# iacopoermacora/Street-sparse-3DGS

Hardware: AMD Instinct MI355X
Metric: fwd+bwd Mpix/s at 1080p (1M Gaussians) (higher is better)
Workload: dtype f32; 1 GPU; rasterizer fwd+bwd, 1000000 Gaussians, SH degree 3, 1920x1080, do_depth; gaussians=1000000, width=1920, height=1080, sh_degree=3, tiles=8160, fwd_segment=2048, parallelism=chunk-per-gpu x1

## Files before the change

### street-sparse-3dgs_amd/csrc/dsort.hip

```cpp
#include "gsr_launch.h"

namespace gsr {

namespace {

constexpr int kDsThreads = 1024;
constexpr int kDsWaves = kDsThreads / kWave;
constexpr int kDsItems = 8;
constexpr int kDsTile = kDsThreads * kDsItems;
constexpr int kRadix = 256;
constexpr int kPasses = 4;
constexpr int kLookWin = 16;
constexpr int kMaxResident = 240;

constexpr int kCtlTicket = 0;
constexpr int kCtlDone = 4;
constexpr int kCtlK = 5;
constexpr int kCtlErr = 6;
constexpr int kCtlAux = 7;
constexpr int kCtlMaxSB = 8;
constexpr int kCtlFwdReady = 9;
constexpr int kCtlLongest = 10;
constexpr int kCtlCulled = 12;
constexpr int kCtlLive = 13;
constexpr int kCtlHead = 16;
constexpr int kUpMax = 128;
__host__ __device__ inline int up_tpb(int nb) { return (nb + kUpMax - 1) / kUpMax; }
__host__ __device__ inline int up_blocks(int nb) { return (nb + up_tpb(nb) - 1) / up_tpb(nb); }
__host__ __device__ inline size_t ctl_status(int nb, int p) { return kCtlHead + (size_t)p * nb * kRadix; }
__host__ __device__ inline size_t ctl_zero_words(int nb) { return ctl_status(nb, kPasses); }
__host__ __device__ inline size_t ctl_bex(int nb) { return ctl_zero_words(nb); }
__host__ __device__ inline size_t ctl_btot(int nb) { return ctl_bex(nb) + nb; }
__host__ __device__ inline size_t ctl_blkhist(int nb) { return (ctl_btot(nb) + kUpMax + 63) / 64 * 64; }
__host__ __device__ inline size_t ctl_words(int nb) { return ctl_blkhist(nb) + (size_t)kUpMax * kPasses * kRadix; }
constexpr int kSpinLimit = 1 << 20;

#ifdef GSR_DS_TRACE
__device__ uint64_t *g_ds_trace;
#define DS_STAMP(kern, slot)                                                                          \
    do {                                                                                              \
        if (threadIdx.x == 0) {                                                                       \
// ... 22 lines not shown
#endif

constexpr uint32_t kFlagAgg = 1u << 30, kFlagInc = 2u << 30, kCountMask = (1u << 30) - 1u;

__device__ __forceinline__ uint32_t ld_agent(const uint32_t *p) {
    return __hip_atomic_load(p, __ATOMIC_RELAXED, __HIP_MEMORY_SCOPE_AGENT);
}
__device__ __forceinline__ void st_agent(uint32_t *p, uint32_t v) {
    __hip_atomic_store(p, v, __ATOMIC_RELAXED, __HIP_MEMORY_SCOPE_AGENT);
}

__device__ __forceinline__ uint32_t below(uint64_t m) {
    return __builtin_amdgcn_mbcnt_hi((uint32_t)(m >> 32), __builtin_amdgcn_mbcnt_lo((uint32_t)m, 0u));
}

__device__ __forceinline__ uint64_t match8(uint32_t d, uint64_t valid) {
    uint64_t m = valid;
#pragma unroll
    for (int b = 0; b < 8; b++) {
        const bool bit = (d >> b) & 1u;
        const uint64_t bb = __ballot(bit);
        m &= bit ? bb : ~bb;
    }
    return m;
}

__device__ __forceinline__ uint32_t wave_incl_scan(uint32_t v, int lane) {
#pragma unroll
    for (int o = 1; o < 64; o <<= 1) {
        const uint32_t t = (uint32_t)__shfl_up((int)v, o, 64);
        if (lane >= o) v += t;
    }
    return v;
}

__device__ __forceinline__ uint32_t scan256_wave(uint32_t *a, int lane) {
    const uint32_t x0 = a[4 * lane], x1 = a[4 * lane + 1], x2 = a[4 * lane + 2], x3 = a[4 * lane + 3];
    const uint32_t s = x0 + x1 + x2 + x3;
    const uint32_t incl = wave_incl_scan(s, lane);
    const uint32_t e = incl - s;
    a[4 * lane] = e;
    a[4 * lane + 1] = e + x0;
    a[4 * lane + 2] = e + x0 + x1;
    a[4 * lane + 3] = e + x0 + x1 + x2;
    return (uint32_t)__shfl((int)incl, 63, 64);
}

__global__ __launch_bounds__(kDsThreads) void dsort_upsweep_kernel(int P, int nb, const uint32_t *__restrict__ keys,
                                                                    const uint32_t *__restrict__ tiles,
                                                                    uint32_t *__restrict__ ctl,
                                                                    uint32_t *__restrict__ host_K) {
    GSR_KS(kKsUpsweep);
    constexpr int kTopCopies = 16;
    __shared__ uint32_t s_hist[kPasses * kRadix];
    __shared__ uint32_t s_top[kTopCopies][kRadix];
    __shared__ uint32_t s_mid[kTopCopies][kRadix];
    __shared__ uint32_t s_wsum[kDsWaves];
    __shared__ uint32_t s_cull;
    const int t = threadIdx.x, w = t >> 6, lane = t & 63;
    const int u = blockIdx.x, tpb = up_tpb(nb);
    DS_STAMP(0, 0);
    s_hist[t] = 0u;
    if (t == 0) s_cull = 0u;
#pragma unroll
    for (int k = 0; k < kTopCopies * kRadix / kDsThreads; k++) {
        (&s_top[0][0])[t + k * kDsThreads] = 0u;
        (&s_mid[0][0])[t + k * kDsThreads] = 0u;
    }
    __syncthreads();
    uint32_t run = 0;
    uint32_t culled = 0;
    const int v1 = min(nb, (u + 1) * tpb);
    for (int v = u * tpb; v < v1; v++) {
        const size_t base = (size_t)v * kDsTile + (size_t)w * kDsItems * kWave;
        uint32_t key[kDsItems], tl[kDsItems];
#pragma unroll
        for (int k = 0; k < kDsItems; k++) {
            const size_t e = base + (size_t)k * kWave + lane;
            key[k] = e < (size_t)P ? keys[e] : 0u;
            tl[k] = e < (size_t)P ? tiles[e] : 0u;
        }
        uint32_t sum = 0;
#pragma unroll
        for (int k = 0; k < kDsItems; k++) {
            const size_t e = base + (size_t)k * kWave + lane;
            const bool cull = e < (size_t)P && key[k] == 0xFFFFFFFFu;
            culled += (uint32_t)__popcll(__ballot(cull));
            if (e < (size_t)P && !cull) {
#pragma unroll
                for (int p = 0; p < kPasses - 2; p++) atomicAdd(&s_hist[p * kRadix + ((key[k] >> (8 * p)) & 0xFFu)], 1u);
                atomicAdd(&s_mid[lane & (kTopCopies - 1)][(key[k] >> 16) & 0xFFu], 1u);
                atomicAdd(&s_top[lane & (kTopCopies - 1)][key[k] >> 24], 1u);
            }
            sum += tl[k];
        }
#pragma unroll
        for (int o = 32; o > 0; o >>= 1) sum += (uint32_t)__shfl_xor((int)sum, o, 64);
        if (lane == 0) s_wsum[w] = sum;
        __syncthreads();
        if (t == 0) {
            ctl[ctl_bex(nb) + v] = run;
#pragma unroll
            for (int k = 0; k < kDsWaves; k++) run += s_wsum[k];
        }
        __syncthreads();
    }
    if (lane == 0 && culled) atomicAdd(&s_cull, culled);
    __syncthreads();
    DS_STAMP(0, 1);
    uint32_t hv = s_hist[t];
    if (t >= (kPasses - 1) * kRadix) {
#pragma unroll
        for (int c = 0; c < kTopCopies; c++) hv += s_top[c][t - (kPasses - 1) * kRadix];
    } else if (t >= (kPasses - 2) * kRadix) {
#pragma unroll
        for (int c = 0; c < kTopCopies; c++) hv += s_mid[c][t - (kPasses - 2) * kRadix];
    }
    ctl[ctl_blkhist(nb) + (size_t)u * kPasses * kRadix + t] = hv;
    if (t == 0) {
        ctl[ctl_btot(nb) + u] = run;
        __hip_atomic_fetch_add(&ctl[kCtlK], run, __ATOMIC_RELAXED, __HIP_MEMORY_SCOPE_AGENT);
        if (s_cull) __hip_atomic_fetch_add(&ctl[kCtlCulled], s_cull, __ATOMIC_RELAXED, __HIP_MEMORY_SCOPE_AGENT);
        const uint32_t done = __hip_atomic_fetch_add(&ctl[kCtlDone], 1u, __ATOMIC_ACQ_REL, __HIP_MEMORY_SCOPE_AGENT);
        if (done == (uint32_t)gridDim.x - 1u && host_K) {
            const uint32_t K = ld_agent(&ctl[kCtlK]);
            __hip_atomic_store(host_K, K, __ATOMIC_RELAXED, __HIP_MEMORY_SCOPE_SYSTEM);
        }
    }
    DS_STAMP(0, 2);
}

template <int kPass>
__global__ __launch_bounds__(kDsThreads) void dsort_pass_kernel(int P, int nb, const uint32_t *__restrict__ kin,
                                                                 uint32_t *__restrict__ kout,
                                                                 const uint32_t *__restrict__ vin,
                                                                 uint32_t *__restrict__ vout, uint32_t *__restrict__ ctl,
                                                                 uint32_t *__restrict__ offsets,
                                                                 const uint32_t *__restrict__ tiles,
                                                                 const uint2 *__restrict__ rect8,
                                                                 const uint32_t *__restrict__ rect4,
                                                                 uint2 *__restrict__ drect,
                                                                 const uint32_t *__restrict__ rin,
                                                                 uint32_t *__restrict__ rout,
                                                                 uint32_t *__restrict__ host_err) {
    GSR_KS(kKsPass0 + kPass);
    constexpr bool kFirst = kPass == 0, kLast = kPass == kPasses - 1;
    const bool carry = GSR_DSORT_CARRY && rect4 != nullptr;
    constexpr int kShift = 8 * kPass;
    __shared__ uint32_t s_key[kDsTile];
    __shared__ uint32_t s_val[kDsTile];
    __shared__ uint32_t s_rc[GSR_DSORT_CARRY ? kDsTile : 1];
    __shared__ uint32_t s_wh[kDsWaves][kRadix];
    __shared__ uint32_t s_gb[4][kRadix];
    __shared__ uint32_t s_bex[kRadix];
    __shared__ uint32_t s_dst[kRadix];
    __shared__ uint32_t s_wsum[kDsWaves];
    __shared__ uint32_t s_v, s_pre, s_nsort;
    const int t = threadIdx.x, w = t >> 6, lane = t & 63;
    DS_STAMP(1 + kPass, 0);
#pragma unroll
    for (int k = 0; k < kDsWaves * kRadix / kDsThreads; k++) (&s_wh[0][0])[t + k * kDsThreads] = 0u;
    const int nbu = up_blocks(nb);
    uint32_t h[kUpMax / 4];
    {
        const uint32_t *bh = ctl + ctl_blkhist(nb) + kPass * kRadix + (t & (kRadix - 1));
#pragma unroll
        for (int q = 0; q < kUpMax / 4; q++) {
            const int j = (t >> 8) + 4 * q;
            h[q] = j < nbu ? bh[(size_t)j * kPasses * kRadix] : 0u;
        }
    }
    uint32_t v = blockIdx.x;
    if (nb > kMaxResident) {
        if (t == 0) s_v = atomicAdd(&ctl[kCtlTicket + kPass], 1u);
        __syncthreads();
        v = s_v;
    } else {
        __builtin_amdgcn_s_waitcnt(0xc07f);
        __builtin_amdgcn_s_barrier();
    }
    const size_t Pn = kFirst ? (size_t)P : (size_t)P - min((size_t)ctl[kCtlCulled], (size_t)P);
    const uint32_t nbv = (uint32_t)((Pn + kDsTile - 1) / kDsTile);
    if (v >= nbv) return;
    DS_STAMP(1 + kPass, 5);
    const int wbase = w * kDsItems * kWave;
    const size_t tile0 = (size_t)v * kDsTile;
    const int n = (int)min((size_t)kDsTile, Pn - tile0);
    uint32_t key[kDsItems], val[kDsItems], tl[kDsItems], rc[kDsItems];
    const uint32_t *rsrc = kFirst ? rect4 : rin;
#pragma unroll
    for (int k = 0; k < kDsItems; k++) {
        const int i = wbase + k * kWave + lane;
        const bool valid = i < n;
        key[k] = valid ? kin[tile0 + i] : 0xFFFFFFFFu;
        val[k] = kFirst ? (uint32_t)(tile0 + i) : (valid ? vin[tile0 + i] : 0u);
        tl[k] = (kFirst && valid) ? tiles[tile0 + i] : 0u;
        rc[k] = (!kFirst && carry && valid) ? rsrc[tile0 + i] : 0u;
    }
    DS_STAMP_AFTER(1 + kPass, 6, key[kDsItems - 1] + val[kDsItems - 1]);
    uint32_t toff[kDsItems];
    if (kFirst) {
        if (w == 0) {
            const int u = (int)v / up_tpb(nb);
            uint32_t c = 0;
#pragma unroll
            for (int q = 0; q < kUpMax / kWave; q++) c += lane + q * kWave < u ? ctl[ctl_btot(nb) + lane + q * kWave] : 0u;
#pragma unroll
            for (int o = 32; o > 0; o >>= 1) c += (uint32_t)__shfl_xor((int)c, o, 64);
            if (lane == 0) s_pre = c + ctl[ctl_bex(nb) + v];
        }
        uint32_t run = 0;
#pragma unroll
        for (int k = 0; k < kDsItems; k++) {
            const uint32_t incl = wave_incl_scan(tl[k], lane);
            toff[k] = run + incl - tl[k];
            run += (uint32_t)__shfl((int)incl, 63, 64);
        }
        if (lane == 0) s_wsum[w] = run;
    }
    uint32_t rk[kDsItems];
#pragma unroll
    for (int k = 0; k < kDsItems; k++) {
        const bool valid = wbase + k * kWave + lane < n && key[k] != 0xFFFFFFFFu;
        const uint32_t d = (key[k] >> kShift) & 0xFFu;
        const uint64_t m = match8(d, __ballot(valid));
        const uint32_t b = below(m);
        const uint32_t old = s_wh[w][d];
        if (valid && b == 0u) s_wh[w][d] = old + (uint32_t)__popcll(m);
        rk[k] = old + b;
    }
    {
        uint32_t c = 0;
#pragma unroll
        for (int q = 0; q < kUpMax / 4; q++) c += h[q];
        s_gb[t >> 8][t & (kRadix - 1)] = c;
    }
    if (kFirst && carry) {
#pragma unroll
        for (int k = 0; k < kDsItems; k++) {
            const int i = wbase + k * kWave + lane;
            rc[k] = i < n ? rsrc[tile0 + i] : 0u;
        }
    }
    __syncthreads();
    DS_STAMP(1 + kPass, 1);
    if (kFirst) {
        uint32_t pre = s_pre;
        for (int k = 0; k < w; k++) pre += s_wsum[k];
#pragma unroll
        for (int k = 0; k < kDsItems; k++) {
            const int i = wbase + k * kWave + lane;
            if (i < n) offsets[tile0 + i] = pre + toff[k];
        }
    }
    uint32_t cnt = 0;
    if (t < kRadix) {
#pragma unroll
        for (int ww = 0; ww < kDsWaves; ww++) {
            const uint32_t c = s_wh[ww][t];
            s_wh[ww][t] = cnt;
            cnt += c;
        }
        uint32_t *st = ctl + ctl_status(nb, kPass);
        st_agent(&st[(size_t)v * kRadix + t], (v == 0 ? kFlagInc : kFlagAgg) | cnt);
        s_bex[t] = cnt;
        s_gb[0][t] += s_gb[1][t] + s_gb[2][t] + s_gb[3][t];
    }
    __syncthreads();
    if (w == 0) {
        const uint32_t nv = scan256_wave(s_bex, lane);
        if (lane == 0) s_nsort = nv;
    }
    if (w == 1) (void)scan256_wave(s_gb[0], lane);
    __syncthreads();
    const int nsort = (int)s_nsort;
    DS_STAMP(1 + kPass, 2);
#pragma unroll
    for (int k = 0; k < kDsItems; k++) {
        const int i = wbase + k * kWave + lane;
        if (i < n && key[k] != 0xFFFFFFFFu) {
            const uint32_t d = (key[k] >> kShift) & 0xFFu;
            const uint32_t lp = s_bex[d] + s_wh[w][d] + rk[k];
            s_key[lp] = key[k];
            s_val[lp] = val[k];
            if (GSR_DSORT_CARRY && carry) s_rc[lp] = rc[k];
        }
    }
    DS_STAMP(1 + kPass, 7);
    if (t < kRadix) {
        const uint32_t *st = ctl + ctl_status(nb, kPass);
        uint32_t excl = 0;
        int spins = 0;
        for (int j = (int)v - 1; j >= 0;) {
            uint32_t s[kLookWin];
#pragma unroll
            for (int q = 0; q < kLookWin; q++)
                s[q] = j - q >= 0 ? ld_agent(&st[(size_t)(j - q) * kRadix + t]) : kFlagInc;
            int q = 0;
            bool inc = false;
// ... 12 lines not shown
                if (++spins > kSpinLimit) {
                    ctl[kCtlErr] = 1u;
                    if (host_err) __hip_atomic_store(host_err, 1u, __ATOMIC_RELAXED, __HIP_MEMORY_SCOPE_SYSTEM);
                    break;
                }
                __builtin_amdgcn_s_sleep(1);
            }
        }
        if (v > 0) st_agent(&ctl[ctl_status(nb, kPass) + (size_t)v * kRadix + t], kFlagInc | (excl + cnt));
        s_dst[t] = s_gb[0][t] + excl - s_bex[t];
    }
    __syncthreads();
    DS_STAMP(1 + kPass, 3);
    for (int i = t; i < nsort; i += kDsThreads) {
        const uint32_t k = s_key[i];
        const uint32_t j = s_dst[(k >> kShift) & 0xFFu] + (uint32_t)i;
        const uint32_t g = s_val[i];
        if (kLast) {
            vout[j] = g;
            if (GSR_DSORT_CARRY && carry) {
                reinterpret_cast<uint32_t *>(drect)[j] = s_rc[i];
            } else if (rect4) {
                reinterpret_cast<uint32_t *>(drect)[j] = rect4[g];
            } else {
                drect[j] = rect8[g];
            }
        } else {
            kout[j] = k;
            vout[j] = g;
            if (GSR_DSORT_CARRY && carry) rout[j] = s_rc[i];
        }
    }
    DS_STAMP(1 + kPass, 4);
}

}

int dsort_blocks(int P) { return (P + kDsTile - 1) / kDsTile; }

size_t dsort_ctrl_words(int P) { return ctl_words(dsort_blocks(P) > 0 ? dsort_blocks(P) : 1); }
size_t dsort_ctrl_zero_words(int P) { return ctl_zero_words(dsort_blocks(P) > 0 ? dsort_blocks(P) : 1); }

void launch_depth_sort(int P, const GeomState &gs, uint32_t *host_K, uint32_t *host_err, hipStream_t s,
                       hipEvent_t k_ready) {
    if (P == 0) return;
    const int nb = dsort_blocks(P);
    hipLaunchKernelGGL(dsort_upsweep_kernel, dim3(up_blocks(nb)), dim3(kDsThreads), 0, s, P, nb, gs.dkey, gs.tiles,
                       gs.ctrl, host_K);
    if (k_ready) (void)hipEventRecord(k_ready, s);
    uint32_t *ra = reinterpret_cast<uint32_t *>(gs.rect8), *rb = ra + P;
    hipLaunchKernelGGL(dsort_pass_kernel<0>, dim3(nb), dim3(kDsThreads), 0, s, P, nb, gs.dkey, gs.dkey_sorted,
                       (const uint32_t *)nullptr, gs.ids, gs.ctrl, gs.offsets, gs.tiles, gs.rect8, gs.rect4, gs.drect,
                       (const uint32_t *)nullptr, ra, host_err);
    hipLaunchKernelGGL(dsort_pass_kernel<1>, dim3(nb), dim3(kDsThreads), 0, s, P, nb, gs.dkey_sorted, gs.dkey, gs.ids,
                       gs.order, gs.ctrl, gs.offsets, gs.tiles, gs.rect8, gs.rect4, gs.drect, ra, rb, host_err);
    hipLaunchKernelGGL(dsort_pass_kernel<2>, dim3(nb), dim3(kDsThreads), 0, s, P, nb, gs.dkey, gs.dkey_sorted, gs.order,
                       gs.ids, gs.ctrl, gs.offsets, gs.tiles, gs.rect8, gs.rect4, gs.drect, rb, ra, host_err);
    hipLaunchKernelGGL(dsort_pass_kernel<3>, dim3(nb), dim3(kDsThreads), 0, s, P, nb, gs.dkey_sorted,
                       (uint32_t *)nullptr, gs.ids, gs.order, gs.ctrl, gs.offsets, gs.tiles, gs.rect8, gs.rect4, gs.drect,
                       ra, (uint32_t *)nullptr, host_err);
}

uint32_t *dsort_K_word(const GeomState &gs) { return gs.ctrl + kCtlK; }
uint32_t *dsort_err_word(const GeomState &gs) { return gs.ctrl + kCtlErr; }
uint32_t *dsort_aux_word(const GeomState &gs) { return gs.ctrl + kCtlAux; }
uint32_t *dsort_maxsb_word(const GeomState &gs) { return gs.ctrl + kCtlMaxSB; }
uint32_t *dsort_fwdready_word(const GeomState &gs) { return gs.ctrl + kCtlFwdReady; }
uint32_t *dsort_longest_words(const GeomState &gs) { return gs.ctrl + kCtlLongest; }
uint32_t *dsort_culled_word(const GeomState &gs) { return gs.ctrl + kCtlCulled; }
uint32_t *dsort_live_words(const GeomState &gs) { return gs.ctrl + kCtlLive; }
int dsort_head_words() { return kCtlHead; }

GSR_KSTAMP_READER(kstamp_read_dsort)

}
// ... 1 lines not shown
```

### street-sparse-3dgs_amd/csrc/gsr_device.h

```cpp
#pragma once
#include <hip/hip_runtime.h>
#include <stdint.h>

namespace gsr {

constexpr int kTile = 16;
constexpr int kWave = 64;
constexpr int kPixPerLane = kTile * kTile / kWave;

#define GSR_SH_C0 0.28209479177387814f
#define GSR_SH_C1 0.4886025119029199f
#define GSR_SH_C2_0 1.0925484305920792f
#define GSR_SH_C2_1 -1.0925484305920792f
#define GSR_SH_C2_2 0.31539156525252005f
#define GSR_SH_C2_3 -1.0925484305920792f
#define GSR_SH_C2_4 0.5462742152960396f
#define GSR_SH_C3_0 -0.5900435899266435f
#define GSR_SH_C3_1 2.890611442640554f
#define GSR_SH_C3_2 -0.4570457994644658f
#define GSR_SH_C3_3 0.3731763325901154f
#define GSR_SH_C3_4 -0.4570457994644658f
#define GSR_SH_C3_5 1.445305721320277f
#define GSR_SH_C3_6 -0.5900435899266435f

// ... 502 lines not shown
    uint32_t ctrl_zero;
    uint2 *drect;
    uint2 *rect8;
    uint32_t *rect4;
    SBGrid sb;
    uint32_t *sb_cnt_g;
    uint32_t *sb_cnt_i;
    uint32_t *sb_base_g;
    uint32_t *sb_base_i;
    float4 *acc;
    int nacc;
    uint32_t *live_stamp;
    uint32_t *tb_flag;
    uint32_t *tb_items;
    uint32_t *tb_cnt;
};
__host__ __device__ __forceinline__ uint2 unpack_rect4(uint32_t q) {
    return make_uint2((q & 0xFFu) | ((q << 8) & 0xFF0000u), ((q >> 16) & 0xFFu) | ((q >> 8) & 0xFF0000u));
}
__host__ __device__ __forceinline__ const uint32_t *drect4_of(const GeomState &g) {
    return g.rect4 ? reinterpret_cast<const uint32_t *>(g.drect) : nullptr;
}

#ifndef GSR_HOST_WORDS
#define GSR_HOST_WORDS 1
#endif
enum HostWord { kHostK = 0, kHostErr = 1, kHostMaxSB = 2, kHostP1 = 3, kHostSBList = 4, kHostTileList = 5,
                kHostFwdGiveUp = 6, kHostFwdErr = 7, kHostWords = 8 };
struct FwdSpin {
    uint32_t ready, flag;
    uint32_t *host;
};
constexpr uint32_t kFwdReadySpins = 1u << 18;
constexpr uint32_t kFwdFlagSpins = 1u << 22;
constexpr uint32_t kFwdReadyNever = 0xFFFFFFFFu;
struct FrameWords {
    uint32_t *dev_K;
    uint32_t *dev_maxsb;
    uint32_t *host;
};

struct BinningState {
    uint2 *sblist;
// ... 89 lines not shown
```

### street-sparse-3dgs_amd/csrc/gsr_launch.h

```cpp
#pragma once
#include <hip/hip_runtime.h>
#include <stdint.h>
#include <string>
#include "gsr_device.h"
#include "../../include/gsr_train.h"

namespace gsr {

void set_last_error(const std::string &msg);
bool true_scale_gradient();

struct Camera {
    const float *view;
    const float *proj;
    const float *campos;
    float tanx, tany, fx, fy;
    int W, H, gx, gy;
};

struct GaussianInputs {
    int P, D, M;
    const float *means3D, *shs, *colors_precomp, *opacities, *scales, *rotations, *cov3D_precomp;
    float scale_modifier;
    int raw;
// ... 28 lines not shown
    const uint64_t *cell_key;
    const uint32_t *cell_start;
    uint32_t n_cells;
    float lo[3], hi[3];
    float inv_h;
    int32_t n[3];
};
bool gt_grid_of(const void *index, GtGrid *out);
bool gt_thresholds(double thr, float *T, float *reach);
void launch_gt_far_mask(int64_t P, const float *xyz, const GtGrid &g, float T, float reach, const uint8_t *skip,
                        uint8_t *out, hipStream_t s);

int dsort_blocks(int P);
size_t dsort_ctrl_words(int P);
size_t dsort_ctrl_zero_words(int P);
void launch_depth_sort(int P, const GeomState &gs, uint32_t *host_K, uint32_t *host_err, hipStream_t s,
                       hipEvent_t k_ready);
uint32_t *dsort_K_word(const GeomState &gs);
uint32_t *dsort_err_word(const GeomState &gs);
uint32_t *dsort_aux_word(const GeomState &gs);
uint32_t *dsort_maxsb_word(const GeomState &gs);
uint32_t *dsort_fwdready_word(const GeomState &gs);
uint32_t *dsort_longest_words(const GeomState &gs);
int device_cus();
uint32_t *dsort_live_words(const GeomState &gs);
uint32_t *dsort_culled_word(const GeomState &gs);
int dsort_head_words();
SBGrid sb_grid(int gx, int gy, int P);
bool sb_grid_supported(const SBGrid &g);
int sort_cap();
int debug_trace(int64_t *out, int n, int reset);
void launch_binning_count(int P, const Camera &cam, const GeomState &gs, bool index_order, const FrameWords &fw,
// ... 97 lines not shown
```

### street-sparse-3dgs_amd/csrc/rasterizer.hip

```cpp
#include <cstdio>
#include <cstring>
#include <atomic>
#include <chrono>
#include <mutex>
#include <string>
#include <algorithm>
#include <thread>
#include <unordered_map>
#include <vector>

#include "../../include/gsr.h"
#include "../../include/gsr_hier.h"
#include "gsr_launch.h"

using namespace gsr;

namespace gsr {
int device_cus() {
    static int cache[64] = {};
    int dev = 0;
    if (hipGetDevice(&dev) != hipSuccess || dev < 0 || dev >= 64) return 256;
    if (!cache[dev]) {
        int n = 0;
        cache[dev] = hipDeviceGetAttribute(&n, hipDeviceAttributeMultiprocessorCount, dev) == hipSuccess && n > 0 ? n : 256;
// ... 117 lines not shown
    hipStream_t s = nullptr;
    hipEvent_t join = nullptr;
    bool pending = false;
    ~SideJoin() {
        if (pending) (void)hipStreamWaitEvent(s, join, 0);
    }
};

int fail(int code, const std::string &msg) {
    g_err = msg;
    return code;
}

std::atomic<int64_t> g_fwd_giveups{0}, g_kwait_ns{0};
std::atomic<int64_t> g_fsplit_frames{0}, g_tbsplit_frames{0};
constexpr int kFwdStats = 8;
void collect_giveups() {
    if (!g_pinned) return;
    const uint32_t gu = __atomic_exchange_n(&g_pinned[kHostFwdGiveUp], 0u, __ATOMIC_SEQ_CST);
    if (gu && g_fwd_giveups.fetch_add(1) == 0)
        fprintf(stderr, "[gsr] forward split: workers gave up waiting for tile_order (side and main streams not "
                        "concurrent); the frame was completed by the pool's second launch, slower "
                        "(gsr_forward_stats[4] counts such frames)\n");
}
int sticky_sort_error() {
    if (!g_pinned) return GSR_OK;
    collect_giveups();
    const uint32_t e = __atomic_exchange_n(&g_pinned[kHostErr], 0u, __ATOMIC_SEQ_CST);
    const uint32_t fe = __atomic_exchange_n(&g_pinned[kHostFwdErr], 0u, __ATOMIC_SEQ_CST);
    if (e) return fail(GSR_ERR_DEVICE, "depth sort: a lookback spin timed out (this or an earlier frame; its image is NaN)");
    if (fe)
// ... 86 lines not shown
    g.drect = c.take<uint2>(P);
    g.rect8 = c.take<uint2>(P);
    g.rect4 = c.take<uint32_t>(P);
    if (!GSR_RECT4 || gx > 255 || gy > 255) g.rect4 = nullptr;
    g.sb = sb_grid(gx, gy, P);
    g.sb_cnt_g = c.take<uint32_t>((size_t)g.sb.nsb * g.sb.ccols);
    g.sb_cnt_i = c.take<uint32_t>((size_t)g.sb.nsb * g.sb.ccols);
    g.sb_base_g = c.take<uint32_t>((size_t)g.sb.nsb + 1);
    g.sb_base_i = c.take<uint32_t>((size_t)g.sb.nsb + 1);
    g.acc = GSR_PERSISTENT_ACC ? nullptr : c.take<float4>(4 * (size_t)P);
    g.nacc = GSR_PERSISTENT_ACC ? 0 : P;
    g.live_stamp = c.take<uint32_t>(P);
    g.tb_flag = c.take<uint32_t>((size_t)g.sb.nsb + 1);
    g.tb_items = c.take<uint32_t>(kTBMaxItems);
    g.tb_cnt = c.take<uint32_t>((size_t)kTBMaxItems << (2 * g.sb.shift));
    if (bytes) *bytes = align_up(c.off, 256);
    return g;
}

size_t segment_end(int64_t K, uint32_t L, uint32_t Lf) {
    size_t end = ck_offset(K);
    if (L) end += align256(ck_slots(K, L) * (kCkFloats * 256) * 4 + ck_slots(K, L) * 4);
    if (Lf) {
        const FwdSegLayout f = fseg_layout(nullptr, K, L, Lf);
        end = (size_t)reinterpret_cast<uintptr_t>(f.part) + fseg_max_items(K, Lf) * kFwdPartials * 256 * 4;
    }
    return end;
}

BinningState carve_binning(void *base, int64_t K, size_t *bytes, uint32_t L = 0, uint32_t Lf = 0) {
// ... 387 lines not shown
        return fail(GSR_ERR_DEVICE, "no current device");
    const bool defer = GSR_DEFER_K && P > 0 && !debug && g_khint[dev] > 0;
    hipEvent_t k_ready = nullptr;
    if (P > 0) {
        if (!g_pinned) {
            if (hipHostMalloc(reinterpret_cast<void **>(&g_pinned), kHostWords * sizeof(uint32_t),
                              hipHostMallocCoherent) != hipSuccess ||
                hipHostGetDevicePointer(reinterpret_cast<void **>(&g_pinned_dev), g_pinned, 0) != hipSuccess)
                return fail(GSR_ERR_ALLOCATION, "pinned host allocation failed");
            for (int k = 0; k < kHostWords; k++) g_pinned[k] = 0u;
            for (int d = 0; d < kMaxDevicesK; d++) g_long_tile_at[d] = g_long_sb_at[d] = -2 * kSplitMemory;
        }
        if (!g_k_ready[dev] && hipEventCreateWithFlags(&g_k_ready[dev], hipEventDisableTiming) != hipSuccess)
            return fail(GSR_ERR_DEVICE, "event creation failed");
        k_ready = (defer && GSR_K_POLL) ? nullptr : g_k_ready[dev];
        __atomic_store_n(&g_pinned[kHostK], kKPending, __ATOMIC_SEQ_CST);
    }
    const FrameWords fw_local{dsort_K_word(gs), dsort_maxsb_word(gs), g_pinned_dev};
    const FrameWords fw_none{nullptr, nullptr, nullptr};
    const bool sb_order = GSR_FWD_SB_ORDER && P > 0;
    uint32_t *const order_sb = sb_order ? is.tile_ids : nullptr;
    uint32_t *const zero_cls = GSR_BWD_CLS && need_bwd && sb_order ? is.bwd_cnt : nullptr;
    if (local) {
        {
            StageTimer st(1, s);
            launch_binning_count(P, cam, gs, true, fw_local, order_sb, zero_cls, s, false);
            if (k_ready) (void)hipEventRecord(k_ready, s);
        }
        if ((rc = check("binning (counts)", debug, s))) return rc;
    } else if (P > 0) {
        {
            StageTimer st(1, s);
            launch_depth_sort(P, gs, g_pinned_dev + kHostK, g_pinned_dev + kHostErr, s, k_ready);
        }
        if ((rc = check("depth sort", debug, s))) return rc;
    }
    int64_t K = 0;
    uint32_t maxsb = 0;
    bool have_K = P == 0;
    auto read_K = [&]() -> int {
        const auto t_wait = std::chrono::steady_clock::now();
        if (k_ready) {
            if (hipEventSynchronize(k_ready) != hipSuccess) return fail(GSR_ERR_DEVICE, "num_rendered wait failed");
        } else {
            while (__atomic_load_n(&g_pinned[kHostK], __ATOMIC_SEQ_CST) == kKPending) {
                const hipError_t q = hipStreamQuery(s);
                if (q == hipSuccess) break;
                if (q != hipErrorNotReady) return fail(GSR_ERR_DEVICE, "num_rendered wait failed");
// ... 5 lines not shown
                             std::memory_order_relaxed);
        uint32_t k = __atomic_load_n(&g_pinned[kHostK], __ATOMIC_ACQUIRE);
        uint32_t m = __atomic_load_n(&g_pinned[kHostMaxSB], __ATOMIC_ACQUIRE);
        if (k == kKPending) {
            const uint32_t *kw = local ? gs.sb_base_i + gs.sb.nsb : dsort_K_word(gs);
            if (hipMemcpy(&k, kw, sizeof(uint32_t), hipMemcpyDeviceToHost) != hipSuccess ||
                hipMemcpy(&m, dsort_maxsb_word(gs), sizeof(uint32_t), hipMemcpyDeviceToHost) != hipSuccess)
                return fail(GSR_ERR_DEVICE, "num_rendered copy failed");
        }
        if (debug && !local) {
            uint32_t err = 0;
            if (hipMemcpy(&err, dsort_err_word(gs), sizeof(uint32_t), hipMemcpyDeviceToHost) != hipSuccess || err)
                return fail(GSR_ERR_DEVICE, "depth sort: a lookback spin timed out");
        }
        if ((rc = sticky_sort_error())) return rc;
        K = (int64_t)k;
        maxsb = local ? m : 0u;
        have_K = true;
        return GSR_OK;
    };
    auto to_global = [&]() -> int {
        local = false;
        g_fallbacks.fetch_add(1, std::memory_order_relaxed);
        if (hipMemsetAsync(gs.ctrl, 0, sizeof(uint32_t) * (size_t)dsort_head_words(), s) != hipSuccess)
            return fail(GSR_ERR_DEVICE, "depth sort control reset failed");
        {
            StageTimer st(1, s);
            launch_depth_sort(P, gs, nullptr, g_pinned_dev + kHostErr, s, nullptr);
        }
        return check("depth sort", debug, s);
    };
    if (P > 0 && !defer) {
        if ((rc = read_K())) return rc;
        if (local && maxsb > (uint32_t)sort_cap() && (rc = to_global())) return rc;
    }
    if (split && !GSR_COLOR_SERIAL && !color_early && (rc = fork_color(radii))) return rc;
    bool joined = false;
    const uint32_t seg_req = need_bwd && bwd_segments_supported() ? g_bwd_seg.load(std::memory_order_relaxed) : 0u;
    uint32_t fseg_req = fwd_segments_supported() && !sb_order ? g_fwd_seg.load(std::memory_order_relaxed) : 0u;
    uint32_t tb_req = GSR_TB_SPLIT;
    const uint32_t fseg_min = fseg_req ? fseg_min_len(fseg_req) : 0u;
    const FwdSpin spin = fwd_spin(g_pinned_dev);
    if (P > 0) {
// ... 296 lines not shown
    if (L > 0 && !bwd_segments_supported())
        return fail(GSR_ERR_UNSUPPORTED, "backward segments need the class launch order and the 1-row sub-block forward");
    return (int)g_bwd_seg.exchange((uint32_t)L);
}

int gsr_set_binning(int mode) {
    if (mode < 0 || mode > 1) return fail(GSR_ERR_INVALID_ARGUMENT, "gsr_set_binning: mode 0 or 1");
    return g_binning_mode.exchange(mode);
}

int gsr_forward_stats(int64_t *out, int n) {
    if (!out || n < 0) return fail(GSR_ERR_INVALID_ARGUMENT, "NULL stats buffer");
    collect_giveups();
    const int64_t v[kFwdStats] = {g_frames.load(), g_reruns.load(), g_local_frames.load(), g_fallbacks.load(),
                                  g_fwd_giveups.load(), g_kwait_ns.load(), g_fsplit_frames.load(),
                                  g_tbsplit_frames.load()};
    int k = 0;
    for (; k < n && k < kFwdStats; k++) out[k] = v[k];
    return k;
}

int gsr_segment_layout_check(int64_t K, int L, int Lf, int64_t *need, int64_t *have) {
    if (K < 0 || L < 0 || Lf < 0) return fail(GSR_ERR_INVALID_ARGUMENT, "negative size");
    size_t bytes = 0;
    carve_binning(nullptr, K, &bytes, (uint32_t)L, (uint32_t)Lf);
    const size_t end = segment_end(K, (uint32_t)L, (uint32_t)Lf);
    if (need) *need = (int64_t)end;
    if (have) *have = (int64_t)bytes;
    return end <= bytes ? GSR_OK : GSR_ERR_INVALID_ARGUMENT;
}

// ... 74 lines not shown
```

### street-sparse-3dgs_amd/diff_gaussian_rasterization/_C.py

```python
from __future__ import annotations

import ctypes

import torch

from . import _lib

_L = _lib.load()
try:
    from . import _gsr_host as _host
except ImportError as e:
    raise _lib.RasterizerLibraryError(
        f"the rasterizer's host extension _gsr_host.so is missing or stale ({e}); build it with "
        f"`python street-sparse-3dgs_amd/build_hip.py` (or __graft_entry__.build())") from e
_host.bind(_lib.LIB_PATH)

rasterize_gaussians = _host.rasterize_gaussians
rasterize_gaussians_backward = _host.rasterize_gaussians_backward
mark_visible = _host.mark_visible


def _capture_listener(bucket):
    import gsr_dist
    _host.set_grad_provider(gsr_dist.grad_out if bucket is not None else None)
# ... 52 lines not shown


def set_split_gate(enable: bool) -> bool:
    return bool(_L.gsr_set_split_gate(int(bool(enable))))


def set_fwd_spin_limits(ready: int = 0, flag: int = 0) -> None:
    _check(_L.gsr_set_fwd_spin_limits(int(ready), int(flag)), "set_fwd_spin_limits")


def reset_capacity_hint() -> None:
    _L.gsr_reset_capacity_hint()


def forward_stats() -> dict:
    buf = (ctypes.c_int64 * 8)()
    n = _L.gsr_forward_stats(buf, 8)
    keys = ("frames", "reruns", "local_sort", "fallbacks", "fwd_worker_giveups", "k_wait_ns", "fwd_split_frames",
            "tb_split_frames")
    return {k: (int(buf[i]) if n > i else 0) for i, k in enumerate(keys)}


def fwd_pool_stats(reset: bool = False) -> dict:
    buf = (ctypes.c_int64 * 4)()
    n = _L.gsr_fwd_pool_stats(buf, 4, 1 if reset else 0)
    if n < 4:
        raise RuntimeError(f"gsr_fwd_pool_stats failed ({n})")
    ready, flags, total = (buf[i] * 1e-8 for i in range(3))
    return {"ready_wait_s": ready, "flag_wait_s": flags, "total_s": total, "workgroups": int(buf[3]),
            "busy_frac": (1.0 - (ready + flags) / total) if total > 0 else None}


def frame_stats(geomBuffer, P, image_height, image_width) -> dict:
    buf = (ctypes.c_int64 * 4)()
# ... 21 lines not shown
```

Baseline: 3112 Mpix/s.

## Use 9-bit radix digits offset from a key base to skip final sort pass

Switches the depth-key radix sort from 8-bit to 9-bit digits computed relative to a fixed float-bit base (0x3E4CCCCD). The upsweep detects whether any visible key falls outside the narrow top-digit bucket and, if none does, the last pass kernel returns early and pass 2 writes the final order. This removes one full scatter pass in the common case, and the per-block histogram loads are vectorized and interleaved with ranking. The cost is larger radix tables in shared memory, a 9-ballot digit match instead of 8, an extra id buffer, and reliance on depth keys sitting near the base value for the skip to trigger.

Result: faster. 3173 Mpix/s, median of 6 (+2.0%).

```diff
diff --git a/street-sparse-3dgs_amd/csrc/dsort.hip b/street-sparse-3dgs_amd/csrc/dsort.hip
--- a/street-sparse-3dgs_amd/csrc/dsort.hip
+++ b/street-sparse-3dgs_amd/csrc/dsort.hip
@@ -8,10 +8,13 @@
 constexpr int kDsWaves = kDsThreads / kWave;
 constexpr int kDsItems = 8;
 constexpr int kDsTile = kDsThreads * kDsItems;
-constexpr int kRadix = 256;
+constexpr int kDigitBits = 9;
+constexpr int kRadix = 1 << kDigitBits;
 constexpr int kPasses = 4;
 constexpr int kLookWin = 16;
 constexpr int kMaxResident = 240;
+constexpr uint32_t kKeyBase = 0x3E4CCCCDu;
+constexpr uint32_t kTopNarrow = 32u;
 
 constexpr int kCtlTicket = 0;
 constexpr int kCtlDone = 4;
@@ -23,8 +26,13 @@
 constexpr int kCtlLongest = 10;
 constexpr int kCtlCulled = 12;
 constexpr int kCtlLive = 13;
+constexpr int kCtlWide = 15;
 constexpr int kCtlHead = 16;
 constexpr int kUpMax = 128;
+constexpr int kRowVec = 4;
+constexpr int kRowSets = kDsThreads / (kRadix / kRowVec);
+constexpr int kRowLoads = kUpMax / kRowSets;
+constexpr int kRowGroup = 8;
 __host__ __device__ inline int up_tpb(int nb) { return (nb + kUpMax - 1) / kUpMax; }
 __host__ __device__ inline int up_blocks(int nb) { return (nb + up_tpb(nb) - 1) / up_tpb(nb); }
 __host__ __device__ inline size_t ctl_status(int nb, int p) { return kCtlHead + (size_t)p * nb * kRadix; }
@@ -77,13 +85,20 @@
     return __builtin_amdgcn_mbcnt_hi((uint32_t)(m >> 32), __builtin_amdgcn_mbcnt_lo((uint32_t)m, 0u));
 }
 
-__device__ __forceinline__ uint64_t match8(uint32_t d, uint64_t valid) {
+template <int p>
+__device__ __forceinline__ uint32_t digit_of(uint32_t key) {
+    const uint32_t r = key - kKeyBase;
+    if (p < kPasses - 1) return (r >> (kDigitBits * p)) & (uint32_t)(kRadix - 1);
+    return (r >> (kDigitBits * p)) + (key >= kKeyBase ? kTopNarrow : 0u);
+}
+
+__device__ __forceinline__ uint64_t match_digit(uint32_t d, uint64_t valid) {
     uint64_t m = valid;
 #pragma unroll
-    for (int b = 0; b < 8; b++) {
-        const bool bit = (d >> b) & 1u;
-        const uint64_t bb = __ballot(bit);
-        m &= bit ? bb : ~bb;
+    for (int b = 0; b < kDigitBits; b++) {
+        const uint32_t spread = (uint32_t)((int32_t)(d << (31 - b)) >> 31);
+        const uint64_t bb = __ballot(spread != 0u);
+        m &= ~(bb ^ ((uint64_t)spread << 32 | spread));
     }
     return m;
 }
@@ -97,42 +112,48 @@
     return v;
 }
 
-__device__ __forceinline__ uint32_t scan256_wave(uint32_t *a, int lane) {
-    const uint32_t x0 = a[4 * lane], x1 = a[4 * lane + 1], x2 = a[4 * lane + 2], x3 = a[4 * lane + 3];
-    const uint32_t s = x0 + x1 + x2 + x3;
+__device__ __forceinline__ uint32_t scan_radix_wave(uint32_t *a, int lane) {
+    constexpr int kPer = kRadix / kWave;
+    uint32_t x[kPer], s = 0;
+#pragma unroll
+    for (int k = 0; k < kPer; k++) {
+        x[k] = a[kPer * lane + k];
+        s += x[k];
+    }
     const uint32_t incl = wave_incl_scan(s, lane);
-    const uint32_t e = incl - s;
-    a[4 * lane] = e;
-    a[4 * lane + 1] = e + x0;
-    a[4 * lane + 2] = e + x0 + x1;
-    a[4 * lane + 3] = e + x0 + x1 + x2;
+    uint32_t e = incl - s;
+#pragma unroll
+    for (int k = 0; k < kPer; k++) {
+        a[kPer * lane + k] = e;
+        e += x[k];
+    }
     return (uint32_t)__shfl((int)incl, 63, 64);
 }
 
 __global__ __launch_bounds__(kDsThreads) void dsort_upsweep_kernel(int P, int nb, const uint32_t *__restrict__ keys,
                                                                     const uint32_t *__restrict__ tiles,
                                                                     uint32_t *__restrict__ ctl,
-                                                                    uint32_t *__restrict__ host_K) {
+                                                                    uint32_t *__restrict__ host_K,
+                                                                    uint32_t *__restrict__ host_wide) {
     GSR_KS(kKsUpsweep);
-    constexpr int kTopCopies = 16;
+    constexpr int kMidCopies = 16;
     __shared__ uint32_t s_hist[kPasses * kRadix];
-    __shared__ uint32_t s_top[kTopCopies][kRadix];
-    __shared__ uint32_t s_mid[kTopCopies][kRadix];
+    __shared__ uint32_t s_mid[kMidCopies][kRadix];
     __shared__ uint32_t s_wsum[kDsWaves];
-    __shared__ uint32_t s_cull;
+    __shared__ uint32_t s_cull, s_far;
     const int t = threadIdx.x, w = t >> 6, lane = t & 63;
     const int u = blockIdx.x, tpb = up_tpb(nb);
     DS_STAMP(0, 0);
-    s_hist[t] = 0u;
-    if (t == 0) s_cull = 0u;
-#pragma unroll
-    for (int k = 0; k < kTopCopies * kRadix / kDsThreads; k++) {
-        (&s_top[0][0])[t + k * kDsThreads] = 0u;
-        (&s_mid[0][0])[t + k * kDsThreads] = 0u;
-    }
+#pragma unroll
+    for (int k = 0; k < kPasses * kRadix / kDsThreads; k++) s_hist[t + k * kDsThreads] = 0u;
+    if (t == 0) s_cull = s_far = 0u;
+#pragma unroll
+    for (int k = 0; k < kMidCopies * kRadix / kDsThreads; k++) (&s_mid[0][0])[t + k * kDsThreads] = 0u;
     __syncthreads();
     uint32_t run = 0;
     uint32_t culled = 0;
+    uint32_t near = 0;
+    bool far = false;
     const int v1 = min(nb, (u + 1) * tpb);
     for (int v = u * tpb; v < v1; v++) {
         const size_t base = (size_t)v * kDsTile + (size_t)w * kDsItems * kWave;
@@ -148,13 +169,18 @@
         for (int k = 0; k < kDsItems; k++) {
             const size_t e = base + (size_t)k * kWave + lane;
             const bool cull = e < (size_t)P && key[k] == 0xFFFFFFFFu;
+            const bool vis = e < (size_t)P && !cull;
+            const uint32_t top = digit_of<3>(key[k]);
+            const uint64_t nearm = __ballot(vis && top == kTopNarrow);
             culled += (uint32_t)__popcll(__ballot(cull));
-            if (e < (size_t)P && !cull) {
-#pragma unroll
-                for (int p = 0; p < kPasses - 2; p++) atomicAdd(&s_hist[p * kRadix + ((key[k] >> (8 * p)) & 0xFFu)], 1u);
-                atomicAdd(&s_mid[lane & (kTopCopies - 1)][(key[k] >> 16) & 0xFFu], 1u);
-                atomicAdd(&s_top[lane & (kTopCopies - 1)][key[k] >> 24], 1u);
+            near += (uint32_t)__popcll(nearm);
+            if (vis) {
+                atomicAdd(&s_hist[digit_of<0>(key[k])], 1u);
+                atomicAdd(&s_hist[kRadix + digit_of<1>(key[k])], 1u);
+                atomicAdd(&s_mid[lane & (kMidCopies - 1)][digit_of<2>(key[k])], 1u);
+                if (top != kTopNarrow) atomicAdd(&s_hist[3 * kRadix + top], 1u);
             }
+            far = far || __ballot(vis) != nearm;
             sum += tl[k];
         }
 #pragma unroll
@@ -168,26 +194,33 @@
         }
         __syncthreads();
     }
-    if (lane == 0 && culled) atomicAdd(&s_cull, culled);
+    if (lane == 0) {
+        if (culled) atomicAdd(&s_cull, culled);
+        if (near) atomicAdd(&s_hist[3 * kRadix + kTopNarrow], near);
+        if (far) s_far = 1u;
+    }
     __syncthreads();
     DS_STAMP(0, 1);
-    uint32_t hv = s_hist[t];
-    if (t >= (kPasses - 1) * kRadix) {
-#pragma unroll
-        for (int c = 0; c < kTopCopies; c++) hv += s_top[c][t - (kPasses - 1) * kRadix];
-    } else if (t >= (kPasses - 2) * kRadix) {
-#pragma unroll
-        for (int c = 0; c < kTopCopies; c++) hv += s_mid[c][t - (kPasses - 2) * kRadix];
-    }
-    ctl[ctl_blkhist(nb) + (size_t)u * kPasses * kRadix + t] = hv;
+#pragma unroll
+    for (int k = 0; k < kPasses * kRadix / kDsThreads; k++) {
+        const int i = t + k * kDsThreads;
+        uint32_t hv = s_hist[i];
+        if (i >= 2 * kRadix && i < 3 * kRadix) {
+#pragma unroll
+            for (int c = 0; c < kMidCopies; c++) hv += s_mid[c][i - 2 * kRadix];
+        }
+        ctl[ctl_blkhist(nb) + (size_t)u * kPasses * kRadix + i] = hv;
+    }
     if (t == 0) {
         ctl[ctl_btot(nb) + u] = run;
         __hip_atomic_fetch_add(&ctl[kCtlK], run, __ATOMIC_RELAXED, __HIP_MEMORY_SCOPE_AGENT);
         if (s_cull) __hip_atomic_fetch_add(&ctl[kCtlCulled], s_cull, __ATOMIC_RELAXED, __HIP_MEMORY_SCOPE_AGENT);
+        if (s_far) __hip_atomic_fetch_or(&ctl[kCtlWide], 1u, __ATOMIC_RELAXED, __HIP_MEMORY_SCOPE_AGENT);
         const uint32_t done = __hip_atomic_fetch_add(&ctl[kCtlDone], 1u, __ATOMIC_ACQ_REL, __HIP_MEMORY_SCOPE_AGENT);
         if (done == (uint32_t)gridDim.x - 1u && host_K) {
             const uint32_t K = ld_agent(&ctl[kCtlK]);
-            __hip_atomic_store(host_K, K, __ATOMIC_RELAXED, __HIP_MEMORY_SCOPE_SYSTEM);
+            if (host_wide) __hip_atomic_store(host_wide, ld_agent(&ctl[kCtlWide]), __ATOMIC_RELAXED, __HIP_MEMORY_SCOPE_SYSTEM);
+            __hip_atomic_store(host_K, K, __ATOMIC_RELEASE, __HIP_MEMORY_SCOPE_SYSTEM);
         }
     }
     DS_STAMP(0, 2);
@@ -197,7 +230,8 @@
 __global__ __launch_bounds__(kDsThreads) void dsort_pass_kernel(int P, int nb, const uint32_t *__restrict__ kin,
                                                                  uint32_t *__restrict__ kout,
                                                                  const uint32_t *__restrict__ vin,
-                                                                 uint32_t *__restrict__ vout, uint32_t *__restrict__ ctl,
+                                                                 uint32_t *__restrict__ vout,
+                                                                 uint32_t *__restrict__ order, uint32_t *__restrict__ ctl,
                                                                  uint32_t *__restrict__ offsets,
                                                                  const uint32_t *__restrict__ tiles,
                                                                  const uint2 *__restrict__ rect8,
@@ -207,14 +241,16 @@
                                                                  uint32_t *__restrict__ rout,
                                                                  uint32_t *__restrict__ host_err) {
     GSR_KS(kKsPass0 + kPass);
-    constexpr bool kFirst = kPass == 0, kLast = kPass == kPasses - 1;
+    constexpr bool kFirst = kPass == 0;
+    const bool wide = kPass >= 2 && ctl[kCtlWide] != 0u;
+    if (kPass == kPasses - 1 && !wide) return;
+    const bool last = kPass == kPasses - 1 || (kPass == kPasses - 2 && !wide);
     const bool carry = GSR_DSORT_CARRY && rect4 != nullptr;
-    constexpr int kShift = 8 * kPass;
     __shared__ uint32_t s_key[kDsTile];
     __shared__ uint32_t s_val[kDsTile];
     __shared__ uint32_t s_rc[GSR_DSORT_CARRY ? kDsTile : 1];
     __shared__ uint32_t s_wh[kDsWaves][kRadix];
-    __shared__ uint32_t s_gb[4][kRadix];
+    __shared__ __attribute__((aligned(16))) uint32_t s_gb[kRowSets][kRadix];
     __shared__ uint32_t s_bex[kRadix];
     __shared__ uint32_t s_dst[kRadix];
     __shared__ uint32_t s_wsum[kDsWaves];
@@ -224,15 +260,25 @@
 #pragma unroll
     for (int k = 0; k < kDsWaves * kRadix / kDsThreads; k++) (&s_wh[0][0])[t + k * kDsThreads] = 0u;
     const int nbu = up_blocks(nb);
-    uint32_t h[kUpMax / 4];
-    {
-        const uint32_t *bh = ctl + ctl_blkhist(nb) + kPass * kRadix + (t & (kRadix - 1));
-#pragma unroll
-        for (int q = 0; q < kUpMax / 4; q++) {
-            const int j = (t >> 8) + 4 * q;
-            h[q] = j < nbu ? bh[(size_t)j * kPasses * kRadix] : 0u;
-        }
-    }
+    const uint4 *bh = reinterpret_cast<const uint4 *>(ctl + ctl_blkhist(nb) + kPass * kRadix) + (t & (kRadix / kRowVec - 1));
+    const auto row = [&](int q) {
+        const int j = t / (kRadix / kRowVec) + kRowSets * q;
+        return j < nbu ? bh[(size_t)j * (kPasses * kRadix / kRowVec)] : make_uint4(0u, 0u, 0u, 0u);
+    };
+    constexpr int kRowGroups = kRowLoads / kRowGroup, kRowEvery = kDsItems / kRowGroups;
+    static_assert(kRowLoads % kRowGroup == 0 && kDsItems % kRowGroups == 0, "row groups spread over the ranked items");
+    uint4 h[kRowGroup], gsum = make_uint4(0u, 0u, 0u, 0u);
+    const auto sum_rows = [&]() {
+#pragma unroll
+        for (int q = 0; q < kRowGroup; q++) {
+            gsum.x += h[q].x;
+            gsum.y += h[q].y;
+            gsum.z += h[q].z;
+            gsum.w += h[q].w;
+        }
+    };
+#pragma unroll
+    for (int q = 0; q < kRowGroup; q++) h[q] = row(q);
     uint32_t v = blockIdx.x;
     if (nb > kMaxResident) {
         if (t == 0) s_v = atomicAdd(&ctl[kCtlTicket + kPass], 1u);
@@ -249,19 +295,16 @@
     const int wbase = w * kDsItems * kWave;
     const size_t tile0 = (size_t)v * kDsTile;
     const int n = (int)min((size_t)kDsTile, Pn - tile0);
-    uint32_t key[kDsItems], val[kDsItems], tl[kDsItems], rc[kDsItems];
-    const uint32_t *rsrc = kFirst ? rect4 : rin;
+    uint32_t key[kDsItems], val[kDsItems], tl[kDsItems];
 #pragma unroll
     for (int k = 0; k < kDsItems; k++) {
         const int i = wbase + k * kWave + lane;
         const bool valid = i < n;
         key[k] = valid ? kin[tile0 + i] : 0xFFFFFFFFu;
-        val[k] = kFirst ? (uint32_t)(tile0 + i) : (valid ? vin[tile0 + i] : 0u);
+        val[k] = (!kFirst && valid) ? vin[tile0 + i] : 0u;
         tl[k] = (kFirst && valid) ? tiles[tile0 + i] : 0u;
-        rc[k] = (!kFirst && carry && valid) ? rsrc[tile0 + i] : 0u;
     }
     DS_STAMP_AFTER(1 + kPass, 6, key[kDsItems - 1] + val[kDsItems - 1]);
-    uint32_t toff[kDsItems];
     if (kFirst) {
         if (w == 0) {
             const int u = (int)v / up_tpb(nb);
@@ -276,7 +319,7 @@
 #pragma unroll
         for (int k = 0; k < kDsItems; k++) {
             const uint32_t incl = wave_incl_scan(tl[k], lane);
-            toff[k] = run + incl - tl[k];
+            s_key[wbase + k * kWave + lane] = run + incl - tl[k];
             run += (uint32_t)__shfl((int)incl, 63, 64);
         }
         if (lane == 0) s_wsum[w] = run;
@@ -285,20 +328,24 @@
 #pragma unroll
     for (int k = 0; k < kDsItems; k++) {
         const bool valid = wbase + k * kWave + lane < n && key[k] != 0xFFFFFFFFu;
-        const uint32_t d = (key[k] >> kShift) & 0xFFu;
-        const uint64_t m = match8(d, __ballot(valid));
+        const uint32_t d = digit_of<kPass>(key[k]) & (uint32_t)(kRadix - 1);
+        const uint64_t m = match_digit(d, __ballot(valid));
         const uint32_t b = below(m);
         const uint32_t old = s_wh[w][d];
         if (valid && b == 0u) s_wh[w][d] = old + (uint32_t)__popcll(m);
         rk[k] = old + b;
-    }
-    {
-        uint32_t c = 0;
-#pragma unroll
-        for (int q = 0; q < kUpMax / 4; q++) c += h[q];
-        s_gb[t >> 8][t & (kRadix - 1)] = c;
-    }
-    if (kFirst && carry) {
+        if ((k + 1) % kRowEvery == 0 && (k + 1) / kRowEvery < kRowGroups) {
+            asm volatile("" ::: "memory");
+            sum_rows();
+#pragma unroll
+            for (int q = 0; q < kRowGroup; q++) h[q] = row((k + 1) / kRowEvery * kRowGroup + q);
+        }
+    }
+    sum_rows();
+    *reinterpret_cast<uint4 *>(&s_gb[t / (kRadix / kRowVec)][kRowVec * (t & (kRadix / kRowVec - 1))]) = gsum;
+    uint32_t rc[kDsItems];
+    if (carry) {
+        const uint32_t *rsrc = kFirst ? rect4 : rin;
 #pragma unroll
         for (int k = 0; k < kDsItems; k++) {
             const int i = wbase + k * kWave + lane;
@@ -313,7 +360,7 @@
 #pragma unroll
         for (int k = 0; k < kDsItems; k++) {
             const int i = wbase + k * kWave + lane;
-            if (i < n) offsets[tile0 + i] = pre + toff[k];
+            if (i < n) offsets[tile0 + i] = pre + s_key[i];
         }
     }
     uint32_t cnt = 0;
@@ -327,25 +374,30 @@
         uint32_t *st = ctl + ctl_status(nb, kPass);
         st_agent(&st[(size_t)v * kRadix + t], (v == 0 ? kFlagInc : kFlagAgg) | cnt);
         s_bex[t] = cnt;
-        s_gb[0][t] += s_gb[1][t] + s_gb[2][t] + s_gb[3][t];
+        uint32_t gb = s_gb[0][t];
+#pragma unroll
+        for (int q = 1; q < kRowSets; q++) gb += s_gb[q][t];
+        s_gb[0][t] = gb;
     }
     __syncthreads();
     if (w == 0) {
-        const uint32_t nv = scan256_wave(s_bex, lane);
+        const uint32_t nv = scan_radix_wave(s_bex, lane);
         if (lane == 0) s_nsort = nv;
     }
-    if (w == 1) (void)scan256_wave(s_gb[0], lane);
+    if (w == 1) (void)scan_radix_wave(s_gb[0], lane);
     __syncthreads();
     const int nsort = (int)s_nsort;
     DS_STAMP(1 + kPass, 2);
+    int wb = wbase + lane;
+    asm volatile("" : "+v"(wb));
 #pragma unroll
     for (int k = 0; k < kDsItems; k++) {
-        const int i = wbase + k * kWave + lane;
+        const int i = wb + k * kWave;
         if (i < n && key[k] != 0xFFFFFFFFu) {
-            const uint32_t d = (key[k] >> kShift) & 0xFFu;
+            const uint32_t d = digit_of<kPass>(key[k]) & (uint32_t)(kRadix - 1);
             const uint32_t lp = s_bex[d] + s_wh[w][d] + rk[k];
             s_key[lp] = key[k];
-            s_val[lp] = val[k];
+            s_val[lp] = kFirst ? (uint32_t)tile0 + (uint32_t)i : val[k];
             if (GSR_DSORT_CARRY && carry) s_rc[lp] = rc[k];
         }
     }
@@ -388,10 +440,10 @@
     DS_STAMP(1 + kPass, 3);
     for (int i = t; i < nsort; i += kDsThreads) {
         const uint32_t k = s_key[i];
-        const uint32_t j = s_dst[(k >> kShift) & 0xFFu] + (uint32_t)i;
+        const uint32_t j = s_dst[digit_of<kPass>(k) & (uint32_t)(kRadix - 1)] + (uint32_t)i;
         const uint32_t g = s_val[i];
-        if (kLast) {
-            vout[j] = g;
+        if (last) {
+            order[j] = g;
             if (GSR_DSORT_CARRY && carry) {
                 reinterpret_cast<uint32_t *>(drect)[j] = s_rc[i];
             } else if (rect4) {
@@ -415,24 +467,25 @@
 size_t dsort_ctrl_words(int P) { return ctl_words(dsort_blocks(P) > 0 ? dsort_blocks(P) : 1); }
 size_t dsort_ctrl_zero_words(int P) { return ctl_zero_words(dsort_blocks(P) > 0 ? dsort_blocks(P) : 1); }
 
-void launch_depth_sort(int P, const GeomState &gs, uint32_t *host_K, uint32_t *host_err, hipStream_t s,
-                       hipEvent_t k_ready) {
+void launch_depth_sort(int P, const GeomState &gs, uint32_t *host_K, uint32_t *host_wide, uint32_t *host_err,
+                       hipStream_t s, hipEvent_t k_ready) {
     if (P == 0) return;
     const int nb = dsort_blocks(P);
     hipLaunchKernelGGL(dsort_upsweep_kernel, dim3(up_blocks(nb)), dim3(kDsThreads), 0, s, P, nb, gs.dkey, gs.tiles,
-                       gs.ctrl, host_K);
+                       gs.ctrl, host_K, host_wide);
     if (k_ready) (void)hipEventRecord(k_ready, s);
     uint32_t *ra = reinterpret_cast<uint32_t *>(gs.rect8), *rb = ra + P;
     hipLaunchKernelGGL(dsort_pass_kernel<0>, dim3(nb), dim3(kDsThreads), 0, s, P, nb, gs.dkey, gs.dkey_sorted,
-                       (const uint32_t *)nullptr, gs.ids, gs.ctrl, gs.offsets, gs.tiles, gs.rect8, gs.rect4, gs.drect,
-                       (const uint32_t *)nullptr, ra, host_err);
+                       (const uint32_t *)nullptr, gs.ids, (uint32_t *)nullptr, gs.ctrl, gs.offsets, gs.tiles, gs.rect8,
+                       gs.rect4, gs.drect, (const uint32_t *)nullptr, ra, host_err);
     hipLaunchKernelGGL(dsort_pass_kernel<1>, dim3(nb), dim3(kDsThreads), 0, s, P, nb, gs.dkey_sorted, gs.dkey, gs.ids,
-                       gs.order, gs.ctrl, gs.offsets, gs.tiles, gs.rect8, gs.rect4, gs.drect, ra, rb, host_err);
-    hipLaunchKernelGGL(dsort_pass_kernel<2>, dim3(nb), dim3(kDsThreads), 0, s, P, nb, gs.dkey, gs.dkey_sorted, gs.order,
-                       gs.ids, gs.ctrl, gs.offsets, gs.tiles, gs.rect8, gs.rect4, gs.drect, rb, ra, host_err);
+                       gs.ids2, (uint32_t *)nullptr, gs.ctrl, gs.offsets, gs.tiles, gs.rect8, gs.rect4, gs.drect, ra,
+                       rb, host_err);
+    hipLaunchKernelGGL(dsort_pass_kernel<2>, dim3(nb), dim3(kDsThreads), 0, s, P, nb, gs.dkey, gs.dkey_sorted, gs.ids2,
+                       gs.ids, gs.order, gs.ctrl, gs.offsets, gs.tiles, gs.rect8, gs.rect4, gs.drect, rb, ra, host_err);
     hipLaunchKernelGGL(dsort_pass_kernel<3>, dim3(nb), dim3(kDsThreads), 0, s, P, nb, gs.dkey_sorted,
-                       (uint32_t *)nullptr, gs.ids, gs.order, gs.ctrl, gs.offsets, gs.tiles, gs.rect8, gs.rect4, gs.drect,
-                       ra, (uint32_t *)nullptr, host_err);
+                       (uint32_t *)nullptr, gs.ids, (uint32_t *)nullptr, gs.order, gs.ctrl, gs.offsets, gs.tiles,
+                       gs.rect8, gs.rect4, gs.drect, ra, (uint32_t *)nullptr, host_err);
 }
 
 uint32_t *dsort_K_word(const GeomState &gs) { return gs.ctrl + kCtlK; }
diff --git a/street-sparse-3dgs_amd/csrc/gsr_device.h b/street-sparse-3dgs_amd/csrc/gsr_device.h
--- a/street-sparse-3dgs_amd/csrc/gsr_device.h
+++ b/street-sparse-3dgs_amd/csrc/gsr_device.h
@@ -540,6 +540,7 @@
     uint32_t *tb_flag;
     uint32_t *tb_items;
     uint32_t *tb_cnt;
+    uint32_t *ids2;
 };
 __host__ __device__ __forceinline__ uint2 unpack_rect4(uint32_t q) {
     return make_uint2((q & 0xFFu) | ((q << 8) & 0xFF0000u), ((q >> 16) & 0xFFu) | ((q >> 8) & 0xFF0000u));
@@ -552,7 +553,7 @@
 #define GSR_HOST_WORDS 1
 #endif
 enum HostWord { kHostK = 0, kHostErr = 1, kHostMaxSB = 2, kHostP1 = 3, kHostSBList = 4, kHostTileList = 5,
-                kHostFwdGiveUp = 6, kHostFwdErr = 7, kHostWords = 8 };
+                kHostFwdGiveUp = 6, kHostFwdErr = 7, kHostWide = 8, kHostWords = 9 };
 struct FwdSpin {
     uint32_t ready, flag;
     uint32_t *host;
diff --git a/street-sparse-3dgs_amd/csrc/gsr_launch.h b/street-sparse-3dgs_amd/csrc/gsr_launch.h
--- a/street-sparse-3dgs_amd/csrc/gsr_launch.h
+++ b/street-sparse-3dgs_amd/csrc/gsr_launch.h
@@ -66,8 +66,8 @@
 int dsort_blocks(int P);
 size_t dsort_ctrl_words(int P);
 size_t dsort_ctrl_zero_words(int P);
-void launch_depth_sort(int P, const GeomState &gs, uint32_t *host_K, uint32_t *host_err, hipStream_t s,
-                       hipEvent_t k_ready);
+void launch_depth_sort(int P, const GeomState &gs, uint32_t *host_K, uint32_t *host_wide, uint32_t *host_err,
+                       hipStream_t s, hipEvent_t k_ready);
 uint32_t *dsort_K_word(const GeomState &gs);
 uint32_t *dsort_err_word(const GeomState &gs);
 uint32_t *dsort_aux_word(const GeomState &gs);
diff --git a/street-sparse-3dgs_amd/csrc/rasterizer.hip b/street-sparse-3dgs_amd/csrc/rasterizer.hip
--- a/street-sparse-3dgs_amd/csrc/rasterizer.hip
+++ b/street-sparse-3dgs_amd/csrc/rasterizer.hip
@@ -155,7 +155,8 @@
 
 std::atomic<int64_t> g_fwd_giveups{0}, g_kwait_ns{0};
 std::atomic<int64_t> g_fsplit_frames{0}, g_tbsplit_frames{0};
-constexpr int kFwdStats = 8;
+std::atomic<int64_t> g_sort_wide_frames{0}, g_sort_late_pass{0};
+constexpr int kFwdStats = 10;
 void collect_giveups() {
     if (!g_pinned) return;
     const uint32_t gu = __atomic_exchange_n(&g_pinned[kHostFwdGiveUp], 0u, __ATOMIC_SEQ_CST);
@@ -272,6 +273,7 @@
     g.tb_flag = c.take<uint32_t>((size_t)g.sb.nsb + 1);
     g.tb_items = c.take<uint32_t>(kTBMaxItems);
     g.tb_cnt = c.take<uint32_t>((size_t)kTBMaxItems << (2 * g.sb.shift));
+    g.ids2 = c.take<uint32_t>(P);
     if (bytes) *bytes = align_up(c.off, 256);
     return g;
 }
@@ -689,6 +691,7 @@
         if (!g_k_ready[dev] && hipEventCreateWithFlags(&g_k_ready[dev], hipEventDisableTiming) != hipSuccess)
             return fail(GSR_ERR_DEVICE, "event creation failed");
         k_ready = (defer && GSR_K_POLL) ? nullptr : g_k_ready[dev];
+        __atomic_store_n(&g_pinned[kHostWide], 0u, __ATOMIC_RELAXED);
         __atomic_store_n(&g_pinned[kHostK], kKPending, __ATOMIC_SEQ_CST);
     }
     const FrameWords fw_local{dsort_K_word(gs), dsort_maxsb_word(gs), g_pinned_dev};
@@ -706,7 +709,8 @@
     } else if (P > 0) {
         {
             StageTimer st(1, s);
-            launch_depth_sort(P, gs, g_pinned_dev + kHostK, g_pinned_dev + kHostErr, s, k_ready);
+            launch_depth_sort(P, gs, g_pinned_dev + kHostK, g_pinned_dev + kHostWide, g_pinned_dev + kHostErr, s,
+                              k_ready);
         }
         if ((rc = check("depth sort", debug, s))) return rc;
     }
@@ -742,6 +746,8 @@
                 return fail(GSR_ERR_DEVICE, "depth sort: a lookback spin timed out");
         }
         if ((rc = sticky_sort_error())) return rc;
+        if (__atomic_load_n(&g_pinned[kHostWide], __ATOMIC_RELAXED))
+            g_sort_wide_frames.fetch_add(1, std::memory_order_relaxed);
         K = (int64_t)k;
         maxsb = local ? m : 0u;
         have_K = true;
@@ -754,7 +760,7 @@
             return fail(GSR_ERR_DEVICE, "depth sort control reset failed");
         {
             StageTimer st(1, s);
-            launch_depth_sort(P, gs, nullptr, g_pinned_dev + kHostErr, s, nullptr);
+            launch_depth_sort(P, gs, nullptr, nullptr, g_pinned_dev + kHostErr, s, nullptr);
         }
         return check("depth sort", debug, s);
     };
@@ -1081,7 +1087,7 @@
     collect_giveups();
     const int64_t v[kFwdStats] = {g_frames.load(), g_reruns.load(), g_local_frames.load(), g_fallbacks.load(),
                                   g_fwd_giveups.load(), g_kwait_ns.load(), g_fsplit_frames.load(),
-                                  g_tbsplit_frames.load()};
+                                  g_tbsplit_frames.load(), g_sort_wide_frames.load(), g_sort_late_pass.load()};
     int k = 0;
     for (; k < n && k < kFwdStats; k++) out[k] = v[k];
     return k;
diff --git a/street-sparse-3dgs_amd/diff_gaussian_rasterization/_C.py b/street-sparse-3dgs_amd/diff_gaussian_rasterization/_C.py
--- a/street-sparse-3dgs_amd/diff_gaussian_rasterization/_C.py
+++ b/street-sparse-3dgs_amd/diff_gaussian_rasterization/_C.py
@@ -90,10 +90,10 @@
 
 
 def forward_stats() -> dict:
-    buf = (ctypes.c_int64 * 8)()
-    n = _L.gsr_forward_stats(buf, 8)
+    buf = (ctypes.c_int64 * 10)()
+    n = _L.gsr_forward_stats(buf, 10)
     keys = ("frames", "reruns", "local_sort", "fallbacks", "fwd_worker_giveups", "k_wait_ns", "fwd_split_frames",
-            "tb_split_frames")
+            "tb_split_frames", "sort_wide_frames", "sort_late_pass")
     return {k: (int(buf[i]) if n > i else 0) for i, k in enumerate(keys)}
 
 
```
